# mako443/Text2Pos-CVPR2022

Measured on AMD Instinct MI355X. Metric: cells+queries encoded/sec and top-k retrieval QPS, 256-pt cells, 12k-cell DB, higher is better.
Workload: dtype f16x3 (fp32 operands split hi+lo into fp16, 3 f16 MFMAs, fp32 accumulate; fp32-class error) for the encoders / f64 MFMA for the ranking

## Files before the change

include/t2p.h:

```cpp
#ifndef T2P_H
#define T2P_H
#include <stddef.h>
#include <stdint.h>

#ifdef __cplusplus
extern "C" {
#endif

#define T2P_ABI_VERSION 29
#define T2P_DEFAULT_CHUNK_OBJECTS 65000
#define T2P_MAX_CHUNK_OBJECTS 65535
#define T2P_TUNING_MASK 0x1
#define T2P_E_ARG (-1)
#define T2P_E_WORKSPACE (-2)
#define T2P_E_UNSUPPORTED (-3)

typedef void* t2p_stream_t;

int t2p_abi_version(void);
const char* t2p_last_error(void);

typedef struct t2p_cell_weights {
    const float* sa_w1[3];
    const float* sa_b1[3];
    const float* sa_w2[3];
    const float* sa_b2[3];
    const float* ga_w1;
    const float* ga_b1;
    const float* ga_w2;
    const float* ga_b2;
    const float* lin1_w;
    const float* lin1_b;
    const float* lin2_w;
    const float* lin2_b;
    const float* pn_w;
    const float* pn_b;
    const float* col_w1;
    const float* col_b1;
    const float* col_w2;
    const float* col_b2;
    const float* pos_w1;
    const float* pos_b1;
    const float* pos_w2;
    const float* pos_b2;
    const float* merge_w;
    const float* merge_b;
    const float* g_wp;
    const float* g_bp;
    const float* g_wq;
    const float* g_w2;
    const float* g_b2;
    const float* lin_w1;
    const float* lin_b1;
    const float* lin_w2;
    const float* lin_b2;
    const void* sa_w2_x3[3];
    const void* ga_w2_x3;
    const float* sa_b2_x3[3];
    float sa_w2_scale[3];
    const void* lin1_x3;
    const void* lin2_x3;
    const void* merge_x3;
    const void* pn_x3;
    const void* g_wp_x3;
    const void* g_wq_x3;
    float lin1_scale, lin2_scale, merge_scale, pn_scale, g_wp_scale, g_wq_scale;
    const void* sa_w1_x3[3];
    const void* ga_w1_x3;
    const float* class_embedding;
    const float* color_embedding;
    float ga_w1_l1;
    float ga_b1_absmax;
    float sa_wp_l1[3];
    float sa_a1_l1;
    float sa_b1_absmax;
    const void* g_w2_x3;
} t2p_cell_weights;

typedef struct t2p_cell_config {
    int32_t n_pts;
    int32_t embed_dim;
    int32_t pointnet_features;
    int32_t use_class;
    int32_t use_color;
    int32_t use_position;
    int32_t self_loops;
    int32_t knn_k;
    int32_t variation;
    float radius[3];
    int32_t chunk_objects;
    int32_t precision;
    int32_t class_embed;
    int32_t color_embed;
    const int32_t* class_idx;
    const int32_t* color_idx;
// ... 159 lines not shown
```

text2pos-cvpr2022_amd/build.py:

```python
import os
import subprocess
import sys
from concurrent.futures import ThreadPoolExecutor

HERE = os.path.dirname(os.path.abspath(__file__))
CSRC = os.path.join(HERE, "csrc")
OBJ = os.path.join(CSRC, "_obj")
LIB = os.path.join(HERE, "libt2p_hip.so")
SOURCES = ["api.hip", "sample_group.hip", "small_kernels.hip", "tg_gemm.hip", "tg_gemm_tn.hip", "tg_gemm_x3.hip", "train_gemm.hip", "ws_gemm.hip", "ga2.hip", "ws_sa.hip", "sa_rows.hip", "sa3.hip", "sa_points.hip", "sa_x3.hip", "lstm.hip", "train_ops.hip", "sim_topk.hip", "match.hip", "classify.hip"]
HEADERS = [os.path.join(CSRC, "t2p_common.h"), os.path.join(HERE, "..", "include", "t2p.h")]
FLAGS = ["--offload-arch=gfx950", "-O3", "-std=c++17", "-fPIC", "-ffp-contract=off", "-Wall", "-Wno-unused-function"]


def _hipcc():
    for c in (os.environ.get("HIPCC"), "/opt/rocm/bin/hipcc", "hipcc"):
        if c and (os.path.sep not in c or os.path.exists(c)):
            return c
    raise RuntimeError("hipcc not found")


def _stale(target, deps):
    if not os.path.exists(target):
        return True
    t = os.path.getmtime(target)
    return any(os.path.getmtime(d) > t for d in deps)


def build_variant(name: str, defines, verbose: bool = False) -> str:
    global OBJ, LIB
    saved = (OBJ, LIB)
    OBJ, LIB = os.path.join(CSRC, "_obj_" + name), os.path.join(HERE, f"libt2p_hip_{name}.so")
    try:
        return build_hip(force=False, verbose=verbose, extra_flags=tuple("-D" + d for d in defines))
    finally:
        OBJ, LIB = saved


def build_hip(force: bool = False, verbose: bool = False, extra_flags=()) -> str:
    os.makedirs(OBJ, exist_ok=True)
    hipcc = _hipcc()
    jobs = []
    for s in SOURCES:
        src = os.path.join(CSRC, s)
        obj = os.path.join(OBJ, s.replace(".hip", ".o"))
        if force or _stale(obj, [src] + HEADERS):
            jobs.append([hipcc, *FLAGS, *extra_flags, "-c", src, "-o", obj])

    def run(cmd):
        if verbose:
            print(" ".join(cmd), flush=True)
        r = subprocess.run(cmd, capture_output=True, text=True)
        if r.returncode != 0:
            raise RuntimeError("hipcc failed: %s\n%s\n%s" % (" ".join(cmd), r.stdout, r.stderr))
        if verbose and r.stderr.strip():
            print(r.stderr)

    with ThreadPoolExecutor(max_workers=min(4, max(1, len(jobs)))) as ex:
        list(ex.map(run, jobs))
    objs = [os.path.join(OBJ, s.replace(".hip", ".o")) for s in SOURCES]
    if force or jobs or _stale(LIB, objs):
        run([hipcc, "--offload-arch=gfx950", "-shared", "-fPIC", "-Wl,--no-undefined", "-o", LIB, *objs])
    return LIB


def build_peaks() -> str:
    src = os.path.join(HERE, "..", "profiles", "microbench", "peaks.hip")
    lib = os.path.join(HERE, "..", "profiles", "microbench", "libt2p_peaks.so")
    if _stale(lib, [src]):
        r = subprocess.run([_hipcc(), "--offload-arch=gfx950", "-O3", "-std=c++17", "-fPIC", "-shared", "-o", lib, src],
                           capture_output=True, text=True)
        if r.returncode != 0:
            raise RuntimeError("hipcc failed on peaks.hip:\n" + r.stderr)
    return os.path.abspath(lib)


def build_host_ext() -> str:
    import sysconfig
    src = os.path.join(CSRC, "host_ext.c")
    lib = os.path.join(HERE, "_t2p_host" + (sysconfig.get_config_var("EXT_SUFFIX") or ".so"))
    if _stale(lib, [src]):
        cc = os.environ.get("CC") or "gcc"
        r = subprocess.run([cc, "-O3", "-std=gnu11", "-fPIC", "-shared", "-Wall", "-I" + sysconfig.get_paths()["include"], "-o", lib, src,
                            "-lpthread", "-lm"], capture_output=True, text=True)
        if r.returncode != 0:
            raise RuntimeError("building _t2p_host failed:\n" + r.stderr)
    return lib


if __name__ == "__main__":
    if "--variant" in sys.argv:
        i = sys.argv.index("--variant")
        print(build_variant(sys.argv[i + 1], sys.argv[i + 2:]))
# ... 5 lines not shown
```

text2pos-cvpr2022_amd/csrc/api.hip:

```cpp
#include <stdarg.h>
#include <stdlib.h>
#include <string.h>

#include <mutex>
#include <set>
#include <utility>

#include "../../include/t2p.h"
#include "t2p_common.h"

namespace t2p {

static thread_local char g_err[512] = "";

void set_error(const char* fmt, ...) {
    va_list ap;
    va_start(ap, fmt);
    vsnprintf(g_err, sizeof(g_err), fmt, ap);
    va_end(ap);
}

int num_cus() {
    static int cached = 0;
    if (cached == 0) {
// ... 157 lines not shown
        w.prefix[l] = b.take<int32_t>(n + 1);
        w.bounds[l] = b.take<int32_t>(1024 + 1);
    }
    w.seg_ptr = b.take<int32_t>(nb + 1);
    w.guard = b.take<uint32_t>(G_SLOTS);
    w.pool = b.take<float>(nb * D);
    w.l1 = b.take<float>(nb * D);
    w.l2 = b.take<float>(nb * D);
    if (ws) *ws = w;
    return align_up(b.off, 256);
}

int default_chunk(const t2p_cell_config& cfg) { return cfg.chunk_objects > 0 ? cfg.chunk_objects : T2P_DEFAULT_CHUNK_OBJECTS; }

int check_cfg(const t2p_cell_config* cfg) {
    T2P_CHECK_ARG(cfg != nullptr, "encode_cells: cfg is NULL");
    if (cfg->n_pts < 8 || cfg->n_pts > 256) {
        set_error("encode_cells: n_pts=%d not built (8 <= n_pts <= 256 points per object)", cfg->n_pts);
        return T2P_E_UNSUPPORTED;
    }
    if (cfg->objects_only) {
        if (cfg->embed_dim < 64 || cfg->embed_dim > 512 || cfg->embed_dim % 64 != 0) {
            set_error("encode_cells: objects_only supports embed_dim in {64, 128, ..., 512}, got %d", cfg->embed_dim);
            return T2P_E_UNSUPPORTED;
        }
    } else if (cfg->embed_dim != 256 && cfg->embed_dim != 128 && cfg->embed_dim != 384) {
        set_error("encode_cells: embed_dim=%d not built for the cell head (128, 256, 384; the host pads e.g. 300 to 384)", cfg->embed_dim);
        return T2P_E_UNSUPPORTED;
    }
    T2P_CHECK_ARG(cfg->variation == 0 || cfg->variation == 1, "encode_cells: variation=%d (0 = max, 1 = mean)",
                  cfg->variation);
    if (cfg->variation == 1 && cfg->knn_k != 8) {
        set_error("encode_cells: variation=1 (mean aggregation) is built for knn_k = 8 only, got %d", cfg->knn_k);
        return T2P_E_UNSUPPORTED;
    }
    T2P_CHECK_ARG(cfg->pointnet_features >= 0 && cfg->pointnet_features <= 2, "encode_cells: pointnet_features=%d",
                  cfg->pointnet_features);
    T2P_CHECK_ARG(cfg->use_class || cfg->use_color || cfg->use_position, "encode_cells: use_features is empty");
    T2P_CHECK_ARG(cfg->knn_k >= 1 && cfg->knn_k <= 32, "encode_cells: knn_k=%d outside [1,32]", cfg->knn_k);
    T2P_CHECK_ARG(cfg->precision == 0 || cfg->precision == 1, "encode_cells: precision=%d (0 = fp32, 1 = f16x3)",
                  cfg->precision);
    T2P_CHECK_ARG((cfg->tuning & ~T2P_TUNING_MASK) == 0, "encode_cells: tuning=%#x has bits outside %#x", cfg->tuning, T2P_TUNING_MASK);
    T2P_CHECK_ARG(cfg->chunk_objects >= 0 && cfg->chunk_objects <= T2P_MAX_CHUNK_OBJECTS,
                  "encode_cells: chunk_objects=%d outside [0, %d] (0 = default %d); the workspace takes ~0.6 MB per object of a chunk",
                  cfg->chunk_objects, T2P_MAX_CHUNK_OBJECTS, T2P_DEFAULT_CHUNK_OBJECTS);
    T2P_CHECK_ARG(!cfg->class_embed || cfg->class_idx != nullptr, "encode_cells: class_embed needs class_idx");
    T2P_CHECK_ARG(!cfg->color_embed || cfg->color_idx != nullptr, "encode_cells: color_embed needs color_idx");
    return 0;
}

template <typename T>
int copy_trace(T* dst, const T* src, size_t n, hipStream_t st) {
    if (dst == nullptr || n == 0) return 0;
    hipError_t e = hipMemcpyAsync(dst, src, n * sizeof(T), hipMemcpyDeviceToDevice, st);
    if (e != hipSuccess) {
        set_error("encode_cells: trace copy failed: %s", hipGetErrorString(e));
        return (int)e;
    }
    return 0;
}

int encode_chunk(const float* xyz, const float* rgb, const float* center, const float* mean_rgb,
                 const int32_t* cell_ptr_dev , int32_t o_lo, int64_t n, int64_t nb,
                 int max_cell, const t2p_cell_weights& W, const t2p_cell_config& cfg, float* out,
                 const t2p_cell_trace* tr, int64_t trace_obj0, CellWs& ws, hipStream_t st, bool trunk_only = false) {
    Geo g(cfg.n_pts);
    const int D = cfg.embed_dim;
    uint32_t* guard = (cfg.precision == 1 && cfg.overflow_flag != nullptr) ? ws.guard : nullptr;
    auto gslot = [&](int i) -> uint32_t* { return guard ? guard + i : nullptr; };
    GuardBounds gbounds{};
    for (int l = 0; l < 3; l++) gbounds.wp_l1[l] = W.sa_wp_l1[l];
    gbounds.a1_l1 = W.sa_a1_l1;
    gbounds.a1_bmax = W.sa_b1_absmax;
    gbounds.ga1_l1 = W.ga_w1_l1;
    gbounds.ga1_bmax = W.ga_b1_absmax;
    bool lds_btab[3];
    for (int l = 0; l < 3; l++) lds_btab[l] = cfg.precision == 1 && g.specialised(l);
    const bool sa1_points = lds_btab[0];
    if (trunk_only)
        T2P_TRY(launch_one_cell_index(n, ws.seg_ptr, ws.first, st, guard));
    else
        T2P_TRY(launch_cell_index(cell_ptr_dev, (int)nb, o_lo, ws.seg_ptr, ws.first, st, guard));
    const bool run_pointnet = cfg.use_class && !cfg.class_embed;
    if (run_pointnet) {
    ws.gt.self_loops = cfg.self_loops;
    {
        GroupTables gt = ws.gt;
        const bool want_nbr = tr != nullptr && (tr->nbr[0] || tr->nbr[1] || tr->nbr[2] || tr->cnt[0] || tr->cnt[1] || tr->cnt[2]);
        if (!want_nbr)
            for (int l = 0; l < 3; l++) gt.nbr[l] = gt.cnt[l] = nullptr;
        for (int l = 0; l < 3; l++) {
            const int cf = l == 0 ? 3 : Geo::C[l - 1];
            gt.B[l] = lds_btab[l] ? nullptr : ws.B[l];
            gt.wp[l] = W.sa_w1[l] + (size_t)cf * Geo::H[l];
            gt.H[l] = Geo::H[l];
            gt.tail[l] = ws.F[l];
            gt.ld_tail[l] = Geo::LD[l];
            gt.tail_col0[l] = Geo::C[l];
        }
        gt.tail_rows[2] = g.gp;
        gt.A1 = sa1_points ? nullptr : ws.A[0];
        gt.w1 = W.sa_w1[0];
        gt.b1 = W.sa_b1[0];
        gt.rgb = rgb;
        gt.H1 = Geo::H[0];
        gt.guard = guard;

        T2P_TRY(launch_sample_group(xyz, n, cfg.n_pts, cfg.radius, gt, st));
        if (!(cfg.tuning & 1) && cfg.n_pts == 256)
            T2P_TRY(launch_dedup_rows(xyz, rgb, n, cfg.n_pts, gt.rows[0], gt.n_rows[0], g.nc[0], st));
        SaParams bp[3] = {};
        for (int l = 0; l < 3; l++) {
            bp[l].n_rows = gt.n_rows[l];
            bp[l].n_obj = n;
            bp[l].prefix_ws = ws.prefix[l];
            bp[l].bounds_ws = ws.bounds[l];
            bp[l].W_x3 = cfg.precision == 1 ? W.sa_w2_x3[l] : nullptr;
            bp[l].wp = lds_btab[l] ? W.sa_w1[l] : nullptr;
            bp[l].n_dense = g.nd[l];
            bp[l].n_cent = g.nc[l];
        }
        bp[0].w1 = sa1_points ? W.sa_w1[0] : nullptr;
        T2P_TRY(launch_sa_balance_levels(bp, Geo::H, Geo::C, st));
    }

    for (int l = 0; l < 3; l++) {
        const int H = Geo::H[l], C = Geo::C[l];
        const int cf = l == 0 ? 3 : Geo::C[l - 1];
        const float* pos_src = l == 0 ? xyz : ws.F[l - 1];
        const int ld_pos = l == 0 ? 3 : Geo::LD[l - 1];
        const int pos_col0 = l == 0 ? 0 : Geo::C[l - 1];
        if (l != 0) {
            WsParams p{};
            p.A = ws.F[l - 1];
            p.lda = Geo::LD[l - 1];
            p.k_live = Geo::C[l - 1] + 4;
            p.W = W.sa_w1[l];
            p.W_x3 = cfg.precision == 1 ? W.sa_w1_x3[l] : nullptr;
            p.ldw = H;
            p.bias = W.sa_b1[l];
            p.out = ws.A[l];
            p.ldo = H;
            p.relu = 0;
            p.M = n * g.nd[l];
            p.amax_out = gslot(l == 1 ? G_A2 : G_A3);
            T2P_TRY(launch_ws(WS_DENSE_STORE, Geo::LD[l - 1] - (cfg.precision == 1 ? 16 : 0), H, p, st));
        }
        SaParams p{};
        p.A = ws.A[l];
        p.Bc = ws.B[l];
        p.wp = lds_btab[l] ? W.sa_w1[l] + (size_t)cf * Geo::H[l] : nullptr;
        p.W = W.sa_w2[l];
        p.W_x3 = cfg.precision == 1 ? W.sa_w2_x3[l] : nullptr;
        p.bias = cfg.precision == 1 ? W.sa_b2_x3[l] : W.sa_b2[l];
        p.out_scale = cfg.precision == 1 ? 1.0f / W.sa_w2_scale[l] : 1.0f;
        p.out = ws.F[l];
        p.ldo = Geo::LD[l];
        p.rows = ws.gt.rows[l];
        p.n_rows = ws.gt.n_rows[l];
        p.first = ws.first;
        p.fps_idx = ws.gt.fps_idx[l];
        p.pos_src = pos_src;
        p.ld_pos = ld_pos;
        p.pos_col0 = pos_col0;
        if (l == 0 && sa1_points) {
            p.feat_src = rgb;
            p.w1 = W.sa_w1[0];
            p.b1 = W.sa_b1[0];
        }
        p.n_dense = g.nd[l];
        p.n_cent = g.nc[l];
        p.n_obj = n;
        p.prefix_ws = ws.prefix[l];
        p.bounds_ws = ws.bounds[l];
        p.balanced = 1;
        p.amax_out = gslot(G_F1 + l);
        if (l == 2) p.out_rows = g.gp;
        T2P_TRY(launch_ws_sa(H, C, p, st));
    }
    {
        WsParams p{};
        p.A = ws.F[2];
        p.lda = Geo::LD[2];
        p.W = W.ga_w1;
        p.W_x3 = cfg.precision == 1 ? W.ga_w1_x3 : nullptr;
        p.ldw = 512;
        p.bias = W.ga_b1;
        p.out = ws.gh;
        _Float16* gh_hi = (_Float16*)ws.gh;
        _Float16* gh_lo = gh_hi + (size_t)gh_rows(n, g) * 512;
        if (cfg.precision == 1) {
            p.out_hi = gh_hi;
            p.out_lo = gh_lo;
            p.amax_out = gslot(G_GA_H);
        }
        p.ldo = 512;
        p.relu = 1;
        p.M = n * g.gp;
        T2P_TRY(launch_ws(WS_DENSE_STORE, Geo::LD[2] - (cfg.precision == 1 ? 16 : 0), 512, p, st));
        WsParams q{};
        q.A = ws.gh;
        if (cfg.precision == 1) {
            q.A_hi = gh_hi;
            q.A_lo = gh_lo;
        }
        q.lda = 512;
        q.W = W.ga_w2;
        q.W_x3 = cfg.precision == 1 ? W.ga_w2_x3 : nullptr;
        q.ldw = 1024;
        q.bias = W.ga_b2;
        q.out = ws.f0;
        q.ldo = 1024;
        q.relu = 1;
        q.M = n * g.gp;
        q.group_rows = g.gp;
        T2P_TRY(launch_ws(WS_DENSE_GROUPMAX, 512, 1024, q, st));
    }
    if (cfg.precision == 1 && W.lin1_x3 && W.lin2_x3) {
        T2P_TRY(launch_gemm_x3(ws.f0, 1024, W.lin1_x3, W.lin1_scale, W.lin1_b, ws.f1, 512, 0, n, 1024, 512, 1, st, nullptr, 0, gslot(G_PN_F0)));
        T2P_TRY(launch_gemm_x3(ws.f1, 512, W.lin2_x3, W.lin2_scale, W.lin2_b, ws.f2, 256, 0, n, 512, 256, 1, st, nullptr, 0, gslot(G_PN_F1)));
    } else {
        T2P_TRY(launch_gemm(ws.f0, 1024, W.lin1_w, W.lin1_b, ws.f1, 512, 0, n, 1024, 512, 1, st));
        T2P_TRY(launch_gemm(ws.f1, 512, W.lin2_w, W.lin2_b, ws.f2, 256, 0, n, 512, 256, 1, st));
    }
    }
    if (trunk_only) {
        T2P_TRY(copy_trace(tr->features0, ws.f0, (size_t)n * 1024, st));
        T2P_TRY(copy_trace(tr->features1, ws.f1, (size_t)n * 512, st));
        T2P_TRY(copy_trace(tr->features2, ws.f2, (size_t)n * 256, st));
        T2P_TRY(launch_guard_check(guard, cfg.overflow_flag, gbounds, st));
        return 0;
    }
    const int nfeat = (cfg.use_class ? 1 : 0) + (cfg.use_color ? 1 : 0) + (cfg.use_position ? 1 : 0);
    const int ldcat = nfeat * D;
    int slot = 0;
    if (cfg.use_class && cfg.class_embed) {
        T2P_TRY(launch_gather_rownorm(W.class_embedding, cfg.class_idx + o_lo, n, D, ws.cat, ldcat, slot * D, st));
        slot++;
    } else if (cfg.use_class) {
        const float* fin = cfg.pointnet_features == 0 ? ws.f0 : (cfg.pointnet_features == 1 ? ws.f1 : ws.f2);
        const int kin = cfg.pointnet_features == 0 ? 1024 : (cfg.pointnet_features == 1 ? 512 : 256);
        if (cfg.precision == 1 && W.pn_x3)
            T2P_TRY(launch_gemm_x3(fin, kin, W.pn_x3, W.pn_scale, W.pn_b, ws.P, D, 0, n, kin, D, 1, st, nullptr, 0,
                                          gslot(G_PN_F0 + cfg.pointnet_features)));
        else
            T2P_TRY(launch_gemm(fin, kin, W.pn_w, W.pn_b, ws.P, D, 0, n, kin, D, 1, st));
        T2P_TRY(launch_rownorm(ws.P, D, n, D, ws.cat, ldcat, slot * D, st));
        slot++;
    }
    if (cfg.use_color && cfg.color_embed) {
        T2P_TRY(launch_gather_rownorm(W.color_embedding, cfg.color_idx + o_lo, n, D, ws.cat, ldcat, slot * D, st));
        slot++;
    } else if (cfg.use_color) {
        T2P_TRY(launch_mlp3_norm(mean_rgb, n, W.col_w1, W.col_b1, W.col_w2, W.col_b2, D, ws.cat, ldcat, slot * D, st));
        slot++;
    }
    if (cfg.use_position) {
        T2P_TRY(launch_mlp3_norm(center, n, W.pos_w1, W.pos_b1, W.pos_w2, W.pos_b2, D, ws.cat, ldcat, slot * D, st));
        slot++;
    }
    const float* emb = ws.cat;
    if (nfeat > 1) {
        if (cfg.precision == 1 && W.merge_x3)
            T2P_TRY(launch_gemm_x3(ws.cat, ldcat, W.merge_x3, W.merge_scale, W.merge_b, ws.emb, D, 0, n, ldcat, D, 1, st, nullptr, 0, gslot(G_GEMM_IN)));
        else
            T2P_TRY(launch_gemm(ws.cat, ldcat, W.merge_w, W.merge_b, ws.emb, D, 0, n, ldcat, D, 1, st));
        emb = ws.emb;
    }
    if (cfg.objects_only) {
        T2P_TRY(copy_trace(tr->obj_emb + trace_obj0 * D, emb, (size_t)n * D, st));
        T2P_TRY(launch_guard_check(guard, cfg.overflow_flag, gbounds, st));
        return 0;
    }
    T2P_TRY(launch_rownorm(emb, D, n, D, ws.embn, D, 0, st));
    if (cfg.precision == 1 && W.g_wp_x3 && W.g_wq_x3) {
        T2P_TRY(launch_gemm_x3(ws.embn, D, W.g_wp_x3, W.g_wp_scale, W.g_bp, ws.P, D, 0, n, D, D, 0, st, nullptr, 0, gslot(G_GEMM_IN)));
        T2P_TRY(launch_gemm_x3(ws.embn, D, W.g_wq_x3, W.g_wq_scale, nullptr, ws.Q, D, 0, n, D, D, 0, st, nullptr, 0, gslot(G_GEMM_IN)));
    } else {
        T2P_TRY(launch_gemm(ws.embn, D, W.g_wp, W.g_bp, ws.P, D, 0, n, D, D, 0, st));
        T2P_TRY(launch_gemm(ws.embn, D, W.g_wq, nullptr, ws.Q, D, 0, n, D, D, 0, st));
    }
    T2P_TRY(launch_knn(ws.embn, D, ws.seg_ptr, (int)nb, max_cell, cfg.knn_k, ws.knn, st));
    {
        WsParams p{};
        p.A = ws.Q;
        p.lda = D;
        p.Bc = ws.P;
        p.W = W.g_w2;
        p.W_x3 = cfg.precision == 1 ? W.g_w2_x3 : nullptr;
        p.amax_out = gslot(G_EDGE);
        p.ldw = D;
        p.bias = W.g_b2;
        p.out = ws.x1;
        p.ldo = D;
        p.relu = 1;
        p.knn_group = (n + 31) / 32 < num_cus() ? 8 : 32;
        p.n_groups = (n + p.knn_group - 1) / p.knn_group;
        p.knn_idx = ws.knn;
        p.knn_k = cfg.knn_k;
        p.n_dst = n;
        p.mean = cfg.variation == 1;
        T2P_TRY(launch_ws(WS_EDGE_KNN, D, D, p, st));
    }
    T2P_TRY(launch_segmax(ws.x1, D, ws.seg_ptr, (int)nb, ws.pool, cfg.variation == 1, st));
    T2P_TRY(launch_gemm(ws.pool, D, W.lin_w1, W.lin_b1, ws.l1, D, 0, nb, D, D, 1, st));
    T2P_TRY(launch_gemm(ws.l1, D, W.lin_w2, W.lin_b2, ws.l2, D, 0, nb, D, D, 1, st));
    T2P_TRY(launch_rownorm(ws.l2, D, nb, D, out, D, 0, st));
    T2P_TRY(launch_guard_check(guard, cfg.overflow_flag, gbounds, st));

    if (tr && run_pointnet) {
        for (int l = 0; l < 3; l++) {
            T2P_TRY(copy_trace(tr->fps_idx[l] ? tr->fps_idx[l] + trace_obj0 * g.nc[l] : nullptr, ws.gt.fps_idx[l],
                               (size_t)n * g.nc[l], st));
            T2P_TRY(copy_trace(tr->nbr[l] ? tr->nbr[l] + trace_obj0 * g.nc[l] * 32 : nullptr, ws.gt.nbr[l],
                               (size_t)n * g.nc[l] * 32, st));
            T2P_TRY(copy_trace(tr->cnt[l] ? tr->cnt[l] + trace_obj0 * g.nc[l] : nullptr, ws.gt.cnt[l],
                               (size_t)n * g.nc[l], st));
            if (tr->sa_out[l] && n > 0) {
                const int rows = l == 2 ? g.gp : g.nc[l];
                const size_t ld = Geo::LD[l] * sizeof(float);
                hipError_t e = hipSuccess;
                if (rows == g.nc[l])
                    e = hipMemcpy2DAsync(tr->sa_out[l] + trace_obj0 * g.nc[l] * Geo::LD[l], ld, ws.F[l], ld, (Geo::C[l] + 4) * sizeof(float),
                                         (size_t)n * g.nc[l], hipMemcpyDeviceToDevice, st);
                for (int c = 0; rows != g.nc[l] && c < g.nc[l] && e == hipSuccess; c++)
                    e = hipMemcpy2DAsync(tr->sa_out[l] + (trace_obj0 * g.nc[l] + c) * Geo::LD[l], g.nc[l] * ld, ws.F[l] + (size_t)c * Geo::LD[l],
                                         rows * ld, (Geo::C[l] + 4) * sizeof(float), (size_t)n, hipMemcpyDeviceToDevice, st);
                if (e != hipSuccess) {
                    set_error("encode_cells: trace copy failed: %s", hipGetErrorString(e));
                    return (int)e;
                }
            }
        }
        T2P_TRY(copy_trace(tr->features0 ? tr->features0 + trace_obj0 * 1024 : nullptr, ws.f0, (size_t)n * 1024, st));
        T2P_TRY(copy_trace(tr->features1 ? tr->features1 + trace_obj0 * 512 : nullptr, ws.f1, (size_t)n * 512, st));
        T2P_TRY(copy_trace(tr->features2 ? tr->features2 + trace_obj0 * 256 : nullptr, ws.f2, (size_t)n * 256, st));
    }
    if (tr) {
        T2P_TRY(copy_trace(tr->obj_emb ? tr->obj_emb + trace_obj0 * D : nullptr, emb, (size_t)n * D, st));
        T2P_TRY(copy_trace(tr->knn_idx ? tr->knn_idx + trace_obj0 * cfg.knn_k : nullptr, ws.knn,
                           (size_t)n * cfg.knn_k, st));
    }
    return 0;
}

int64_t next_chunk_end(const int32_t* cp, int64_t c0, int64_t n_cells, int chunk) {
    int64_t c1 = c0 + 1;
    while (c1 < n_cells && (cp[c1 + 1] - cp[c0]) <= chunk) c1++;
    return c1;
}

}
}

using namespace t2p;

extern "C" {

int t2p_abi_version(void) { return T2P_ABI_VERSION; }

void t2p_profile_enable(int on) {
    std::lock_guard<std::mutex> lock(g_prof_mu);
    g_prof_on = on != 0;
// ... 537 lines not shown
```

text2pos-cvpr2022_amd/csrc/t2p_common.h:

```cpp
#pragma once
#include <hip/hip_runtime.h>
#include <stdint.h>
#include <stdio.h>

namespace t2p {

void set_error(const char* fmt, ...);

#define T2P_E_ARG (-1)
#define T2P_E_WORKSPACE (-2)
#define T2P_E_UNSUPPORTED (-3)

#define T2P_CHECK_ARG(cond, ...)                  \
    do {                                          \
        if (!(cond)) {                            \
            ::t2p::set_error(__VA_ARGS__);        \
            return T2P_E_ARG;                     \
        }                                         \
    } while (0)

#define T2P_CHECK_LAUNCH(name)                                                   \
    do {                                                                         \
        hipError_t e__ = hipGetLastError();                                      \
        if (e__ != hipSuccess) {                                                 \
// ... 81 lines not shown
    if ((threadIdx.x & 63) == 0) {
        const uint32_t b = __float_as_uint(m);
        if (b > __atomic_load_n(slot, __ATOMIC_RELAXED)) atomicMax(slot, b);
    }
}
__device__ __forceinline__ void guard_track_bits(uint32_t& acc, int lane_bits ) {
#pragma unroll
    for (int o = 32; o > 0; o >>= 1) {
        const int other = __shfl_xor(lane_bits, o, 64);
        lane_bits = other > lane_bits ? other : lane_bits;
    }
    const uint32_t b = (uint32_t)__builtin_amdgcn_readfirstlane(lane_bits);
    acc = b > acc ? b : acc;
}
#endif
int launch_guard_check(const uint32_t* guard, int32_t* overflow_flag, const GuardBounds& b, hipStream_t st);

struct ProfScope {
    ProfScope(const char* name, hipStream_t st);
    ~ProfScope();
    int slot;
    hipStream_t st;
    void* ev_end;
    int reps;
};
#define T2P_REPEAT(ps) for (int rep_ = (ps).reps; rep_ > 0; --rep_)

struct GroupTables {
    uint8_t* fps_idx[3];
    uint8_t* nbr[3];
    uint8_t* cnt[3];
    uint16_t* rows[3];
    uint16_t* n_rows[3];
    int self_loops;
    int n_dense[3];
    int n_cent[3];
    float* B[3];
    const float* wp[3];
    int H[3];
    float* tail[3];
    int ld_tail[3], tail_col0[3];
    int tail_rows[3];
    float* A1;
    const float* w1;
    const float* b1;
    const float* rgb;
    int H1;
    uint32_t* guard;
};
int launch_sample_group(const float* xyz, int64_t n_obj, int n_pts, const float radius[3], GroupTables gt,
                        hipStream_t st);
int launch_dedup_rows(const float* xyz, const float* rgb, int64_t n_obj, int n_pts, uint16_t* rows, uint16_t* n_rows,
                      int n_cent, hipStream_t st);

int launch_rownorm(const float* in, int ld_in, int64_t n_rows, int dim, float* out, int ld_out, int col0,
                   hipStream_t st);
int launch_gather_rownorm(const float* table, const int32_t* idx, int64_t n_rows, int dim, float* out, int ld_out,
                          int col0, hipStream_t st);
int launch_segmax(const float* in, int dim, const int32_t* seg_ptr, int n_seg, float* out, int mean,
                  hipStream_t st);
int launch_knn(const float* x, int dim, const int32_t* seg_ptr, int n_seg, int max_seg_rows, int k,
               int32_t* out_idx, hipStream_t st);
int launch_mlp3_norm(const float* in3, int64_t n_rows, const float* w1, const float* b1, const float* w2,
                     const float* b2, int D, float* out, int ld_out, int col0, hipStream_t st);
int launch_pack_objects(const float* raw_xyz, const float* raw_rgb, const int32_t* obj_ptr, const int32_t* sample_idx,
                        const float* rot, int64_t n_obj, int n_pts, float* xyz, float* rgb, float* center, float* mean_rgb,
                        hipStream_t st);
int launch_pack_scene(const float* raw_xyz, const float* raw_rgb, const int32_t* obj_ptr, const int32_t* obj_id, const uint64_t* key,
                      const float* scene_center, const float* scene_color, int64_t n_out, int n_pts, float* xyz, float* rgb,
                      float* center, float* mean_rgb, int32_t* idx_out, hipStream_t st);
int launch_pairwise_ranking(const float* scores, int batch, float margin, float* row_loss, float* d_scores, float* row_cnt,
                            hipStream_t st);
int launch_hardest_ranking(const float* scores, int batch, float margin, float* best, int32_t* where, float* d_scores,
                           hipStream_t st);
int launch_cell_index(const int32_t* cell_ptr, int n_cells, int32_t o_lo, int32_t* seg_ptr_local, int32_t* first,
                      hipStream_t st, uint32_t* guard_to_clear = nullptr);

int launch_gemm(const float* A, int lda, const float* W, const float* bias, float* C, int ldc, int c0, int64_t M,
                int K, int N, int relu, hipStream_t st, const float* resid = nullptr, int ldr = 0);
int launch_gemm_skinny(const float* A, int lda, const float* W, float* C, int ldc, int64_t M, int K, int N, hipStream_t st);
int launch_gemm_x3(const float* A, int lda, const void* Wx, float scale, const float* bias, float* C, int ldc, int c0,
                   int64_t M, int K, int N, int relu, hipStream_t st, const float* resid = nullptr, int ldr = 0,
                   uint32_t* amax_in = nullptr );

size_t gemm_tn_workspace_bytes(int64_t M, int K1, int N);
int launch_edge_counts(const uint16_t* rows, const uint16_t* n_rows, const int32_t* first_obj, int64_t n_obj, int n_dense, int n_cent,
                       int self_loops, int32_t* counts, hipStream_t st);
int launch_edge_expand(const uint16_t* rows, const uint16_t* n_rows, const int32_t* first_obj, const int32_t* cent_ptr, int64_t n_obj,
                       int n_dense, int n_cent, int self_loops, int32_t* src, int32_t* dst, hipStream_t st);
size_t linear_wgrad_workspace_bytes(int64_t M, int K1, int N);
int launch_linear_wgrad_f32(const float* dY, int lda, const float* X, int ldb, float* dW, int ldc, float* colsum, int64_t M, int K1, int N,
                            void* ws, size_t ws_bytes, hipStream_t st);
int launch_gemm_tn(const float* A, int lda, const float* B, int ldb, float* C, int ldc, int64_t M, int K1, int N, void* ws,
                   size_t ws_bytes, hipStream_t st);

enum WsMode { WS_DENSE_STORE = 0, WS_DENSE_GROUPMAX = 1, WS_EDGE_KNN = 3 };
struct WsParams {
    const float* A;
    int lda;
    int k_live;
    const float* Bc;
    const float* W;
    int ldw;
    const void* W_x3;
    const void* A_hi;
    const void* A_lo;
    void* out_hi;
    void* out_lo;
    const float* bias;
    float* out;
    int ldo;
    int relu;
    int64_t n_groups;
    int64_t M;
    uint32_t* amax_out;
    const int32_t* knn_idx;
    int knn_k;
    int64_t n_dst;
    int mean;
    int knn_group;
    int group_rows;
};
int launch_ws(int mode, int K, int N, const WsParams& p, hipStream_t st);

struct SaParams {
    const float* A;
    const float* Bc;
    const float* wp;
    const float* W;
    const void* W_x3;
    const float* bias;
    float out_scale;
    float* out;
    int ldo;
    const uint16_t* rows;
    const uint16_t* n_rows;
    const int32_t* first;
    const uint8_t* fps_idx;
    const float* pos_src;
    int ld_pos, pos_col0;
    const float* feat_src;
    const float* w1;
    const float* b1;
    int n_dense, n_cent;
    int64_t n_obj;
    int32_t* prefix_ws;
    int32_t* bounds_ws;
    int balanced;
    uint32_t* amax_out;
    int out_rows;
};
int launch_ws_sa(int H, int C, const SaParams& p, hipStream_t st);
int launch_sa_x3(int H, int C, const SaParams& p, hipStream_t st);
int sa_x3_launch_shape(int H, int C, int64_t n_obj, int* tile_rows, int* n_wg);
bool sa_rows_selected(int H, int C, const SaParams& p);
int launch_sa_rows(int H, int C, const SaParams& p, hipStream_t st);
int sa_rows_launch_shape(int64_t n_obj, int* tile_rows, int* n_wg);
bool sa_points_selected(int H, int C, const SaParams& p);
int launch_sa_points(int H, int C, const SaParams& p, hipStream_t st);
int sa_points_launch_shape(int64_t n_obj, int* tile_rows, int* n_wg);
bool sa3_selected(int H, int C, const SaParams& p);
int launch_sa3(const SaParams& p, hipStream_t st);
int sa3_launch_shape(int64_t n_obj, int* tile_rows, int* n_wg);
int launch_sa_balance_levels(const SaParams p[3], const int H[3], const int C[3], hipStream_t st);

int launch_bilstm_impl(const float* gate_table , const float* whh ,
// ... 43 lines not shown
```

Measured before the change: 151,300.

## Fuse per-object head MLPs, feature merge, norms and P/Q projections into one kernel

Adds a single persistent kernel that runs the whole per-object head in one pass over a row tile kept in LDS as split fp16 hi/lo planes. The fused stages are lin1, lin2, the pointnet projection and row norm, the color and position MLPs with norm, the merge GEMM and norm, and the P/Q projections. It replaces roughly ten separate launches and their global-memory intermediates (f1, f2, cat). It is enabled by default for the fp16x3, D=256 configuration, and tuning bit 4 turns it off. In exchange it needs a large LDS footprint per block, uses one block per CU with many barriers, and has a complex hand-written pipeline that could run slower than the tuned separate GEMMs.

```diff
diff --git a/include/t2p.h b/include/t2p.h
--- a/include/t2p.h
+++ b/include/t2p.h
@@ -10,7 +10,7 @@
 #define T2P_ABI_VERSION 29
 #define T2P_DEFAULT_CHUNK_OBJECTS 65000
 #define T2P_MAX_CHUNK_OBJECTS 65535
-#define T2P_TUNING_MASK 0x1
+#define T2P_TUNING_MASK 0x5
 #define T2P_E_ARG (-1)
 #define T2P_E_WORKSPACE (-2)
 #define T2P_E_UNSUPPORTED (-3)
diff --git a/text2pos-cvpr2022_amd/build.py b/text2pos-cvpr2022_amd/build.py
--- a/text2pos-cvpr2022_amd/build.py
+++ b/text2pos-cvpr2022_amd/build.py
@@ -7,7 +7,7 @@
 CSRC = os.path.join(HERE, "csrc")
 OBJ = os.path.join(CSRC, "_obj")
 LIB = os.path.join(HERE, "libt2p_hip.so")
-SOURCES = ["api.hip", "sample_group.hip", "small_kernels.hip", "tg_gemm.hip", "tg_gemm_tn.hip", "tg_gemm_x3.hip", "train_gemm.hip", "ws_gemm.hip", "ga2.hip", "ws_sa.hip", "sa_rows.hip", "sa3.hip", "sa_points.hip", "sa_x3.hip", "lstm.hip", "train_ops.hip", "sim_topk.hip", "match.hip", "classify.hip"]
+SOURCES = ["api.hip", "sample_group.hip", "small_kernels.hip", "tg_gemm.hip", "tg_gemm_tn.hip", "tg_gemm_x3.hip", "object_head.hip", "train_gemm.hip", "ws_gemm.hip", "ga2.hip", "ws_sa.hip", "sa_rows.hip", "sa3.hip", "sa_points.hip", "sa_x3.hip", "lstm.hip", "train_ops.hip", "sim_topk.hip", "match.hip", "classify.hip"]
 HEADERS = [os.path.join(CSRC, "t2p_common.h"), os.path.join(HERE, "..", "include", "t2p.h")]
 FLAGS = ["--offload-arch=gfx950", "-O3", "-std=c++17", "-fPIC", "-ffp-contract=off", "-Wall", "-Wno-unused-function"]
 
diff --git a/text2pos-cvpr2022_amd/csrc/api.hip b/text2pos-cvpr2022_amd/csrc/api.hip
--- a/text2pos-cvpr2022_amd/csrc/api.hip
+++ b/text2pos-cvpr2022_amd/csrc/api.hip
@@ -263,6 +263,10 @@
     else
         T2P_TRY(launch_cell_index(cell_ptr_dev, (int)nb, o_lo, ws.seg_ptr, ws.first, st, guard));
     const bool run_pointnet = cfg.use_class && !cfg.class_embed;
+    const bool fused_head = !(cfg.tuning & 4) && !trunk_only && !cfg.objects_only && cfg.precision == 1 && D == 256 && run_pointnet &&
+                            cfg.pointnet_features == 2 && cfg.use_color && !cfg.color_embed && cfg.use_position &&
+                            !(tr && (tr->features1 || tr->features2)) && W.lin1_x3 && W.lin2_x3 && W.pn_x3 && W.merge_x3 &&
+                            W.g_wp_x3 && W.g_wq_x3;
     if (run_pointnet) {
     ws.gt.self_loops = cfg.self_loops;
     {
@@ -397,7 +401,8 @@
         q.group_rows = g.gp;
         T2P_TRY(launch_ws(WS_DENSE_GROUPMAX, 512, 1024, q, st));
     }
-    if (cfg.precision == 1 && W.lin1_x3 && W.lin2_x3) {
+    if (fused_head) {
+    } else if (cfg.precision == 1 && W.lin1_x3 && W.lin2_x3) {
         T2P_TRY(launch_gemm_x3(ws.f0, 1024, W.lin1_x3, W.lin1_scale, W.lin1_b, ws.f1, 512, 0, n, 1024, 512, 1, st, nullptr, 0, gslot(G_PN_F0)));
         T2P_TRY(launch_gemm_x3(ws.f1, 512, W.lin2_x3, W.lin2_scale, W.lin2_b, ws.f2, 256, 0, n, 512, 256, 1, st, nullptr, 0, gslot(G_PN_F1)));
     } else {
@@ -414,6 +419,22 @@
     }
     const int nfeat = (cfg.use_class ? 1 : 0) + (cfg.use_color ? 1 : 0) + (cfg.use_position ? 1 : 0);
     const int ldcat = nfeat * D;
+    const float* emb = ws.cat;
+    if (fused_head) {
+        ObjectHeadArgs a{};
+        a.f0 = ws.f0; a.center = center; a.mean_rgb = mean_rgb; a.M = n;
+        a.lin1_x3 = W.lin1_x3; a.lin2_x3 = W.lin2_x3; a.pn_x3 = W.pn_x3; a.merge_x3 = W.merge_x3; a.wp_x3 = W.g_wp_x3; a.wq_x3 = W.g_wq_x3;
+        a.lin1_scale = W.lin1_scale; a.lin2_scale = W.lin2_scale; a.pn_scale = W.pn_scale; a.merge_scale = W.merge_scale;
+        a.wp_scale = W.g_wp_scale; a.wq_scale = W.g_wq_scale;
+        a.lin1_b = W.lin1_b; a.lin2_b = W.lin2_b; a.pn_b = W.pn_b; a.merge_b = W.merge_b; a.bp = W.g_bp;
+        a.col_w1 = W.col_w1; a.col_b1 = W.col_b1; a.col_w2 = W.col_w2; a.col_b2 = W.col_b2;
+        a.pos_w1 = W.pos_w1; a.pos_b1 = W.pos_b1; a.pos_w2 = W.pos_w2; a.pos_b2 = W.pos_b2;
+        a.emb = (tr && tr->obj_emb) ? ws.emb : nullptr;
+        a.embn = ws.embn; a.P = ws.P; a.Q = ws.Q;
+        a.g_f0 = gslot(G_PN_F0); a.g_f1 = gslot(G_PN_F1); a.g_f2 = gslot(G_PN_F2); a.g_in = gslot(G_GEMM_IN);
+        T2P_TRY(launch_object_head(a, st));
+        emb = ws.emb;
+    } else {
     int slot = 0;
     if (cfg.use_class && cfg.class_embed) {
         T2P_TRY(launch_gather_rownorm(W.class_embedding, cfg.class_idx + o_lo, n, D, ws.cat, ldcat, slot * D, st));
@@ -440,7 +461,6 @@
         T2P_TRY(launch_mlp3_norm(center, n, W.pos_w1, W.pos_b1, W.pos_w2, W.pos_b2, D, ws.cat, ldcat, slot * D, st));
         slot++;
     }
-    const float* emb = ws.cat;
     if (nfeat > 1) {
         if (cfg.precision == 1 && W.merge_x3)
             T2P_TRY(launch_gemm_x3(ws.cat, ldcat, W.merge_x3, W.merge_scale, W.merge_b, ws.emb, D, 0, n, ldcat, D, 1, st, nullptr, 0, gslot(G_GEMM_IN)));
@@ -460,6 +480,7 @@
     } else {
         T2P_TRY(launch_gemm(ws.embn, D, W.g_wp, W.g_bp, ws.P, D, 0, n, D, D, 0, st));
         T2P_TRY(launch_gemm(ws.embn, D, W.g_wq, nullptr, ws.Q, D, 0, n, D, D, 0, st));
+    }
     }
     T2P_TRY(launch_knn(ws.embn, D, ws.seg_ptr, (int)nb, max_cell, cfg.knn_k, ws.knn, st));
     {
diff --git a/text2pos-cvpr2022_amd/csrc/object_head.hip b/text2pos-cvpr2022_amd/csrc/object_head.hip
--- /dev/null
+++ b/text2pos-cvpr2022_amd/csrc/object_head.hip
@@ -0,0 +1,420 @@
+#include "t2p_common.h"
+
+namespace t2p {
+namespace {
+
+typedef _Float16 half8 __attribute__((ext_vector_type(8)));
+
+constexpr int NT = 512;
+constexpr int D = 256;
+constexpr int KC = 64;
+constexpr int LDS_ST = KC + 8;
+constexpr int LD1 = 512 + 8;
+constexpr int LD2 = D + 8;
+constexpr int LDY = D + 4;
+
+template <int RT>
+struct OhCfg {
+    static constexpr int MI = RT / 32;
+    static constexpr int FPT = RT * KC / NT;
+    static constexpr size_t kStage = (size_t)2 * 2 * RT * LDS_ST * sizeof(_Float16);
+    static constexpr size_t kPlanes512 = (size_t)2 * RT * LD1 * sizeof(_Float16);
+    static constexpr size_t kPlanes256 = (size_t)2 * RT * LD2 * sizeof(_Float16);
+    static constexpr size_t kOffY = kPlanes256;
+    static constexpr size_t kOffHid = kOffY + (size_t)RT * LDY * sizeof(float);
+    static constexpr size_t kOffSs = kOffHid + (size_t)RT * 64 * sizeof(float);
+    static constexpr size_t kEnd = kOffSs + (size_t)4 * RT * sizeof(float);
+    static constexpr size_t kLds = kEnd > kPlanes512 ? kEnd : kPlanes512;
+    static_assert(kStage <= kPlanes512 && kLds <= 160 * 1024, "object head: LDS plan");
+};
+
+struct OhParams {
+    const float* f0;
+    const float* center;
+    const float* mean_rgb;
+    int64_t M;
+    const _Float16 *lin1, *lin2, *pn, *merge, *wp, *wq;
+    float lin1_is, lin2_is, pn_is, merge_is, wp_is, wq_is;
+    const float *lin1_b, *lin2_b, *pn_b, *merge_b, *bp;
+    const float *col_w1, *col_b1, *col_w2, *col_b2, *pos_w1, *pos_b1, *pos_w2, *pos_b2;
+    float* emb;
+    float *embn, *P, *Q;
+    uint32_t *g_f0, *g_f1, *g_f2, *g_in;
+};
+
+typedef uint32_t u32x4 __attribute__((ext_vector_type(4)));
+__device__ __forceinline__ __amdgpu_buffer_rsrc_t weight_rsrc(const void* base, uint32_t bytes) {
+    return __builtin_amdgcn_make_buffer_rsrc((void*)base, 0, (int)bytes, 0x00020000);
+}
+template <int NJ>
+__device__ __forceinline__ void load_b(half8 (&b)[4][NJ][2], __amdgpu_buffer_rsrc_t w, uint32_t voff, uint32_t soff, uint32_t lo_bytes, int kp) {
+#pragma unroll
+    for (int s = 0; s < 4; s++)
+#pragma unroll
+        for (int j = 0; j < NJ; j++) {
+            const uint32_t so = soff + (uint32_t)j * 64 * kp;
+            b[s][j][0] = __builtin_bit_cast(half8, __builtin_amdgcn_raw_buffer_load_b128(w, voff + s * 32, so, 0));
+            b[s][j][1] = __builtin_bit_cast(half8, __builtin_amdgcn_raw_buffer_load_b128(w, voff + s * 32, so + lo_bytes, 0));
+        }
+}
+
+template <int MI, int NJ>
+__device__ __forceinline__ void mma_group(f32x16 (&acc)[MI][NJ], const _Float16* a, int a_lo, int lda, const half8 (&b)[4][NJ][2]) {
+#pragma unroll
+    for (int s = 0; s < 4; s++) {
+        half8 ah[MI], al[MI];
+#pragma unroll
+        for (int i = 0; i < MI; i++) {
+            const _Float16* p = a + i * 32 * lda + s * 16;
+            ah[i] = *(const half8*)p;
+            al[i] = *(const half8*)(p + a_lo);
+        }
+#pragma unroll
+        for (int i = 0; i < MI; i++)
+#pragma unroll
+            for (int j = 0; j < NJ; j++) {
+                acc[i][j] = __builtin_amdgcn_mfma_f32_32x32x16_f16(ah[i], b[s][j][0], acc[i][j], 0, 0, 0);
+                acc[i][j] = __builtin_amdgcn_mfma_f32_32x32x16_f16(ah[i], b[s][j][1], acc[i][j], 0, 0, 0);
+                acc[i][j] = __builtin_amdgcn_mfma_f32_32x32x16_f16(al[i], b[s][j][0], acc[i][j], 0, 0, 0);
+            }
+    }
+}
+
+template <int MI, int NJ>
+__device__ __forceinline__ void mma_seg(f32x16 (&acc)[MI][NJ], const _Float16* a, int a_lo, int lda, const _Float16* w, uint32_t soff,
+                                        uint32_t lo_bytes, int kp, int groups, int lane) {
+    const uint32_t voff = (uint32_t)((lane & 31) * kp + (lane >> 5) * 8) * 2u;
+    const __amdgpu_buffer_rsrc_t rs = weight_rsrc(w, 2 * lo_bytes);
+    half8 b0[4][NJ][2], b1[4][NJ][2];
+    load_b<NJ>(b0, rs, voff, soff, lo_bytes, kp);
+#pragma unroll 1
+    for (int g = 0; g < groups; g += 2) {
+        load_b<NJ>(b1, rs, voff, soff + (g + 1) * KC * 2, lo_bytes, kp);
+        mma_group<MI, NJ>(acc, a + g * KC, a_lo, lda, b0);
+        if (g + 2 < groups) load_b<NJ>(b0, rs, voff, soff + (g + 2) * KC * 2, lo_bytes, kp);
+        mma_group<MI, NJ>(acc, a + (g + 1) * KC, a_lo, lda, b1);
+    }
+}
+
+template <int MI, int NJ>
+__device__ __forceinline__ void zero_acc(f32x16 (&acc)[MI][NJ]) {
+#pragma unroll
+    for (int i = 0; i < MI; i++)
+#pragma unroll
+        for (int j = 0; j < NJ; j++)
+#pragma unroll
+            for (int e = 0; e < 16; e++) acc[i][j][e] = 0.f;
+}
+
+__device__ __forceinline__ void split_store(_Float16* hi_plane, int lo_off, int idx, float v) {
+    const _Float16 hi = (_Float16)v;
+    hi_plane[idx] = hi;
+    hi_plane[lo_off + idx] = (_Float16)(v - (float)hi);
+}
+
+template <int MI, int NJ>
+__device__ __forceinline__ void epi_planes(const f32x16 (&acc)[MI][NJ], float inv, const float* __restrict__ bias, int n0,
+                                           _Float16* hi_plane, int lo_off, int ld, int rows_live, float& gmax, int lane) {
+    const int h = lane >> 5, l31 = lane & 31;
+#pragma unroll
+    for (int j = 0; j < NJ; j++) {
+        const int col = n0 + j * 32 + l31;
+        const float bv = bias[col];
+#pragma unroll
+        for (int i = 0; i < MI; i++)
+#pragma unroll
+            for (int e = 0; e < 16; e++) {
+                const int r = i * 32 + (e & 3) + 8 * (e >> 2) + 4 * h;
+                const float v = fmaxf(fmaf(acc[i][j][e], inv, bv), 0.f);
+                if (r < rows_live) gmax = fmaxf(gmax, v);
+                split_store(hi_plane, lo_off, r * ld + col, v);
+            }
+    }
+}
+
+template <int MI>
+__device__ __forceinline__ void epi_f32(const f32x16 (&acc)[MI][1], float inv, const float* __restrict__ bias, int n0, float* Y, int lane) {
+    const int h = lane >> 5, l31 = lane & 31;
+    const int col = n0 + l31;
+    const float bv = bias[col];
+#pragma unroll
+    for (int i = 0; i < MI; i++)
+#pragma unroll
+        for (int e = 0; e < 16; e++) {
+            const int r = i * 32 + (e & 3) + 8 * (e >> 2) + 4 * h;
+            Y[r * LDY + col] = fmaxf(fmaf(acc[i][0][e], inv, bv), 0.f);
+        }
+}
+
+template <int RT>
+__device__ __forceinline__ void rownorm_rows(const float* Y, _Float16* hi_plane, int lo_off, int64_t row0, int rows_live, float* raw,
+                                             float* out, float& gmax, int lane, int wave) {
+#pragma unroll 1
+    for (int r = wave; r < RT; r += NT / 64) {
+        const float* x = Y + r * LDY;
+        float xv[D / 64];
+        float ss = 0.f;
+#pragma unroll
+        for (int j = 0; j < D / 64; j++) {
+            xv[j] = x[lane + 64 * j];
+            ss = fmaf(xv[j], xv[j], ss);
+        }
+#pragma unroll
+        for (int off = 32; off >= 1; off >>= 1) ss += __shfl_xor(ss, off, 64);
+        const float nrm = sqrtf(ss);
+        const float den = nrm > 1e-12f ? nrm : 1e-12f;
+        const bool live = r < rows_live;
+#pragma unroll
+        for (int j = 0; j < D / 64; j++) {
+            const float y = xv[j] / den;
+            split_store(hi_plane, lo_off, r * LD2 + lane + 64 * j, y);
+            if (live) {
+                gmax = fmaxf(gmax, fabsf(y));
+                if (raw) raw[(row0 + r) * D + lane + 64 * j] = xv[j];
+                if (out) out[(row0 + r) * D + lane + 64 * j] = y;
+            }
+        }
+    }
+}
+
+template <int RT>
+__device__ __forceinline__ void mlp_hidden(float* hid, const float* __restrict__ in3, const float* __restrict__ w1,
+                                           const float* __restrict__ b1, int64_t row0, int rows_live, int tid) {
+#pragma unroll 1
+    for (int i = tid; i < RT * 64; i += NT) {
+        const int r = i >> 6, u = i & 63;
+        float hv = 0.f;
+        if (r < rows_live) {
+            const float* x = in3 + (row0 + r) * 3;
+            float a = b1[u];
+            a = fmaf(x[0], w1[u], a);
+            a = fmaf(x[1], w1[64 + u], a);
+            a = fmaf(x[2], w1[128 + u], a);
+            hv = fmaxf(a, 0.f);
+        }
+        hid[i] = hv;
+    }
+}
+
+template <int RT>
+__device__ __forceinline__ void mlp_out_norm(const float* hid, float* ss, const float* __restrict__ w2, const float* __restrict__ b2,
+                                             _Float16* hi_plane, int lo_off, int rows_live, float& gmax, int tid) {
+    constexpr int R2 = RT / 2;
+    const int c = tid & (D - 1), r0 = (tid >> 8) * R2, cw = (tid >> 6) & 3;
+    float o[R2];
+    const float bv = b2[c];
+#pragma unroll
+    for (int r = 0; r < R2; r++) o[r] = bv;
+#pragma unroll 1
+    for (int k = 0; k < 64; k += 4) {
+        const float w0 = w2[k * D + c], w1 = w2[(k + 1) * D + c], w2_ = w2[(k + 2) * D + c], w3 = w2[(k + 3) * D + c];
+#pragma unroll
+        for (int r = 0; r < R2; r++) {
+            const f32x4 hv = *(const f32x4*)(hid + (r0 + r) * 64 + k);
+            o[r] = fmaf(hv[0], w0, o[r]);
+            o[r] = fmaf(hv[1], w1, o[r]);
+            o[r] = fmaf(hv[2], w2_, o[r]);
+            o[r] = fmaf(hv[3], w3, o[r]);
+        }
+    }
+#pragma unroll
+    for (int r = 0; r < R2; r++) {
+        o[r] = fmaxf(o[r], 0.f);
+        float v = fmaf(o[r], o[r], 0.f);
+#pragma unroll
+        for (int off = 32; off >= 1; off >>= 1) v += __shfl_xor(v, off, 64);
+        if ((tid & 63) == 0) ss[cw * RT + r0 + r] = v;
+    }
+    __syncthreads();
+#pragma unroll
+    for (int r = 0; r < R2; r++) {
+        const int rr = r0 + r;
+        const float nrm = sqrtf((ss[rr] + ss[RT + rr]) + (ss[2 * RT + rr] + ss[3 * RT + rr]));
+        const float y = o[r] / (nrm > 1e-12f ? nrm : 1e-12f);
+        if (rr < rows_live) gmax = fmaxf(gmax, y);
+        split_store(hi_plane, lo_off, rr * LD2 + c, y);
+    }
+}
+
+template <int RT>
+__global__ __launch_bounds__(NT) void k_object_head(const OhParams p, int64_t n_tiles) {
+    using Cf = OhCfg<RT>;
+    constexpr int MI = Cf::MI, FPT = Cf::FPT, TPR = KC / FPT;
+    extern __shared__ __attribute__((aligned(16))) unsigned char smem[];
+    _Float16* const X = (_Float16*)smem;
+    float* const Y = (float*)(smem + Cf::kOffY);
+    float* const hid = (float*)(smem + Cf::kOffHid);
+    float* const ss = (float*)(smem + Cf::kOffSs);
+    constexpr int ST_PLANE = RT * LDS_ST, P512 = RT * LD1, P256 = RT * LD2;
+
+    const int tid = threadIdx.x;
+    const int wave = __builtin_amdgcn_readfirstlane(tid >> 6);
+    float gmax_f0 = 0.f, gmax_f1 = 0.f, gmax_f2 = 0.f, gmax_in = 0.f;
+
+    for (int64_t tile = blockIdx.x; tile < n_tiles; tile += gridDim.x) {
+        const int64_t row0 = tile * RT;
+        int t = tid;
+        asm volatile("" : "+v"(t));
+        const int lane = t & 63;
+        const int h = lane >> 5, l31 = lane & 31;
+        const int rows_live = (int)((p.M - row0) < RT ? (p.M - row0) : RT);
+
+        f32x16 acc1[MI][2];
+        zero_acc<MI, 2>(acc1);
+        {
+            const int s_row = t / TPR, s_k = (t % TPR) * FPT;
+            const bool a_ok = s_row < rows_live;
+            const float* a_ptr = p.f0 + (row0 + s_row) * 1024 + s_k;
+            const uint32_t w_lo = 512u * 1024 * 2, w0 = (uint32_t)wave * 64 * 1024 * 2;
+            const __amdgpu_buffer_rsrc_t w = weight_rsrc(p.lin1, 2 * w_lo);
+            const uint32_t voff = (uint32_t)(l31 * 1024 + h * 8) * 2u;
+            const _Float16* a_frag = X + l31 * LDS_ST + h * 8;
+            f32x4 ra[FPT / 4];
+            auto stage_load = [&](int c) {
+#pragma unroll
+                for (int i = 0; i < FPT / 4; i++) ra[i] = a_ok ? *(const f32x4*)(a_ptr + c * KC + 4 * i) : f32x4{0.f, 0.f, 0.f, 0.f};
+            };
+            auto stage_store = [&](int buf) {
+                _Float16* base = X + buf * 2 * ST_PLANE + s_row * LDS_ST + s_k;
+#pragma unroll
+                for (int i = 0; i < FPT / 4; i++) {
+                    const f32x4 v = ra[i];
+                    gmax_f0 = fmaxf(fmaxf(gmax_f0, fmaxf(fabsf(v[0]), fabsf(v[1]))), fmaxf(fabsf(v[2]), fabsf(v[3])));
+                    const t2p_fp16x2 h01 = cvt_pk_f16(v[0], v[1]), h23 = cvt_pk_f16(v[2], v[3]);
+                    const t2p_fp16x2 l01 = cvt_pk_f16(v[0] - (float)h01[0], v[1] - (float)h01[1]);
+                    const t2p_fp16x2 l23 = cvt_pk_f16(v[2] - (float)h23[0], v[3] - (float)h23[1]);
+                    uint2 ph, pl;
+                    ph.x = __builtin_bit_cast(uint32_t, h01); ph.y = __builtin_bit_cast(uint32_t, h23);
+                    pl.x = __builtin_bit_cast(uint32_t, l01); pl.y = __builtin_bit_cast(uint32_t, l23);
+                    *(uint2*)(base + 4 * i) = ph;
+                    *(uint2*)(base + ST_PLANE + 4 * i) = pl;
+                }
+            };
+            half8 b0[4][2][2], b1[4][2][2];
+            stage_load(0);
+            load_b<2>(b0, w, voff, w0, w_lo, 1024);
+            stage_store(0);
+            __syncthreads();
+#pragma unroll 1
+            for (int c = 0; c < 1024 / KC; c += 2) {
+                stage_load(c + 1);
+                load_b<2>(b1, w, voff, w0 + (c + 1) * KC * 2, w_lo, 1024);
+                mma_group<MI, 2>(acc1, a_frag, ST_PLANE, LDS_ST, b0);
+                stage_store(1);
+                __syncthreads();
+                const bool more = c + 2 < 1024 / KC;
+                if (more) {
+                    stage_load(c + 2);
+                    load_b<2>(b0, w, voff, w0 + (c + 2) * KC * 2, w_lo, 1024);
+                }
+                mma_group<MI, 2>(acc1, a_frag + 2 * ST_PLANE, ST_PLANE, LDS_ST, b1);
+                if (more) stage_store(0);
+                __syncthreads();
+            }
+            epi_planes<MI, 2>(acc1, p.lin1_is, p.lin1_b, wave * 64, X, P512, LD1, rows_live, gmax_f1, lane);
+        }
+        __syncthreads();
+
+        f32x16 acc[MI][1];
+        zero_acc<MI, 1>(acc);
+        mma_seg<MI, 1>(acc, X + l31 * LD1 + h * 8, P512, LD1, p.lin2, (uint32_t)wave * 32 * 512 * 2, 256u * 512 * 2, 512, 8, lane);
+        __syncthreads();
+        epi_planes<MI, 1>(acc, p.lin2_is, p.lin2_b, wave * 32, X, P256, LD2, rows_live, gmax_f2, lane);
+        mlp_hidden<RT>(hid, p.mean_rgb, p.col_w1, p.col_b1, row0, rows_live, t);
+        __syncthreads();
+
+        const _Float16* a256 = X + l31 * LD2 + h * 8;
+        const uint32_t wn = (uint32_t)wave * 32;
+        zero_acc<MI, 1>(acc);
+        mma_seg<MI, 1>(acc, a256, P256, LD2, p.pn, wn * 256 * 2, 256u * 256 * 2, 256, 4, lane);
+        epi_f32<MI>(acc, p.pn_is, p.pn_b, wave * 32, Y, lane);
+        __syncthreads();
+        rownorm_rows<RT>(Y, X, P256, row0, rows_live, nullptr, nullptr, gmax_in, lane, wave);
+        __syncthreads();
+
+        f32x16 accm[MI][1];
+        zero_acc<MI, 1>(accm);
+        const uint32_t wm = wn * 768 * 2, wm_lo = 256u * 768 * 2;
+        mma_seg<MI, 1>(accm, a256, P256, LD2, p.merge, wm, wm_lo, 768, 4, lane);
+        __syncthreads();
+        mlp_out_norm<RT>(hid, ss, p.col_w2, p.col_b2, X, P256, rows_live, gmax_in, t);
+        mlp_hidden<RT>(hid, p.center, p.pos_w1, p.pos_b1, row0, rows_live, t);
+        __syncthreads();
+        mma_seg<MI, 1>(accm, a256, P256, LD2, p.merge, wm + 256 * 2, wm_lo, 768, 4, lane);
+        __syncthreads();
+        mlp_out_norm<RT>(hid, ss, p.pos_w2, p.pos_b2, X, P256, rows_live, gmax_in, t);
+        __syncthreads();
+        mma_seg<MI, 1>(accm, a256, P256, LD2, p.merge, wm + 512 * 2, wm_lo, 768, 4, lane);
+        epi_f32<MI>(accm, p.merge_is, p.merge_b, wave * 32, Y, lane);
+        __syncthreads();
+        rownorm_rows<RT>(Y, X, P256, row0, rows_live, p.emb, p.embn, gmax_in, lane, wave);
+        __syncthreads();
+
+        {
+            f32x16 accp[MI][2];
+            zero_acc<MI, 2>(accp);
+            const bool is_q = wave >= 4;
+            const int n0 = (wave & 3) * 64;
+            mma_seg<MI, 2>(accp, a256, P256, LD2, is_q ? p.wq : p.wp, (uint32_t)n0 * 256 * 2, 256u * 256 * 2, 256, 4, lane);
+            const float inv = is_q ? p.wq_is : p.wp_is;
+            float* outp = is_q ? p.Q : p.P;
+#pragma unroll
+            for (int j = 0; j < 2; j++) {
+                const int col = n0 + j * 32 + l31;
+                const float bv = is_q ? 0.f : p.bp[col];
+#pragma unroll
+                for (int i = 0; i < MI; i++)
+#pragma unroll
+                    for (int e = 0; e < 16; e++) {
+                        const int r = i * 32 + (e & 3) + 8 * (e >> 2) + 4 * h;
+                        if (r < rows_live) outp[(row0 + r) * D + col] = fmaf(accp[i][j][e], inv, bv);
+                    }
+            }
+        }
+        __syncthreads();
+    }
+    guard_publish_exact(p.g_f0, gmax_f0);
+    guard_publish_exact(p.g_f1, gmax_f1);
+    guard_publish_exact(p.g_f2, gmax_f2);
+    guard_publish_exact(p.g_in, gmax_in);
+}
+
+}
+
+int launch_object_head(const ObjectHeadArgs& a, hipStream_t st) {
+    T2P_CHECK_ARG(a.f0 && a.center && a.mean_rgb && a.embn && a.P && a.Q && a.lin1_x3 && a.lin2_x3 && a.pn_x3 && a.merge_x3 && a.wp_x3 &&
+                      a.wq_x3 && a.lin1_b && a.lin2_b && a.pn_b && a.merge_b && a.bp && a.col_w1 && a.col_b1 && a.col_w2 && a.col_b2 &&
+                      a.pos_w1 && a.pos_b1 && a.pos_w2 && a.pos_b2,
+                  "object_head: NULL argument");
+    T2P_CHECK_ARG(a.lin1_scale > 0.f && a.lin2_scale > 0.f && a.pn_scale > 0.f && a.merge_scale > 0.f && a.wp_scale > 0.f && a.wq_scale > 0.f,
+                  "object_head: weight image scales must be positive");
+    T2P_CHECK_ARG(((((uintptr_t)a.f0) | ((uintptr_t)a.lin1_x3) | ((uintptr_t)a.lin2_x3) | ((uintptr_t)a.pn_x3) | ((uintptr_t)a.merge_x3) |
+                    ((uintptr_t)a.wp_x3) | ((uintptr_t)a.wq_x3)) & 15) == 0,
+                  "object_head: f0 and the weight images must be 16-byte aligned");
+    if (a.M == 0) return 0;
+    OhParams p{};
+    p.f0 = a.f0; p.center = a.center; p.mean_rgb = a.mean_rgb; p.M = a.M;
+    p.lin1 = (const _Float16*)a.lin1_x3; p.lin2 = (const _Float16*)a.lin2_x3; p.pn = (const _Float16*)a.pn_x3;
+    p.merge = (const _Float16*)a.merge_x3; p.wp = (const _Float16*)a.wp_x3; p.wq = (const _Float16*)a.wq_x3;
+    p.lin1_is = 1.0f / a.lin1_scale; p.lin2_is = 1.0f / a.lin2_scale; p.pn_is = 1.0f / a.pn_scale;
+    p.merge_is = 1.0f / a.merge_scale; p.wp_is = 1.0f / a.wp_scale; p.wq_is = 1.0f / a.wq_scale;
+    p.lin1_b = a.lin1_b; p.lin2_b = a.lin2_b; p.pn_b = a.pn_b; p.merge_b = a.merge_b; p.bp = a.bp;
+    p.col_w1 = a.col_w1; p.col_b1 = a.col_b1; p.col_w2 = a.col_w2; p.col_b2 = a.col_b2;
+    p.pos_w1 = a.pos_w1; p.pos_b1 = a.pos_b1; p.pos_w2 = a.pos_w2; p.pos_b2 = a.pos_b2;
+    p.emb = a.emb; p.embn = a.embn; p.P = a.P; p.Q = a.Q;
+    p.g_f0 = a.g_f0; p.g_f1 = a.g_f1; p.g_f2 = a.g_f2; p.g_in = a.g_in;
+    ProfScope ps_("object_head", st);
+    const int64_t tiles32 = (a.M + 31) / 32, tiles64 = (a.M + 63) / 64;
+    if (tiles32 < num_cus()) {
+        T2P_TRY(reserve_lds((const void*)k_object_head<32>, OhCfg<32>::kLds, "object_head"));
+        hipLaunchKernelGGL(k_object_head<32>, dim3((unsigned)tiles32), dim3(NT), OhCfg<32>::kLds, st, p, tiles32);
+    } else {
+        T2P_TRY(reserve_lds((const void*)k_object_head<64>, OhCfg<64>::kLds, "object_head"));
+        const unsigned grid = (unsigned)(tiles64 < num_cus() ? tiles64 : num_cus());
+        hipLaunchKernelGGL(k_object_head<64>, dim3(grid), dim3(NT), OhCfg<64>::kLds, st, p, tiles64);
+    }
+    T2P_CHECK_LAUNCH("object_head");
+    return 0;
+}
+
+}
diff --git a/text2pos-cvpr2022_amd/csrc/t2p_common.h b/text2pos-cvpr2022_amd/csrc/t2p_common.h
--- a/text2pos-cvpr2022_amd/csrc/t2p_common.h
+++ b/text2pos-cvpr2022_amd/csrc/t2p_common.h
@@ -187,6 +187,21 @@
 int launch_gemm_x3(const float* A, int lda, const void* Wx, float scale, const float* bias, float* C, int ldc, int c0,
                    int64_t M, int K, int N, int relu, hipStream_t st, const float* resid = nullptr, int ldr = 0,
                    uint32_t* amax_in = nullptr );
+
+struct ObjectHeadArgs {
+    const float* f0;
+    const float* center;
+    const float* mean_rgb;
+    int64_t M;
+    const void *lin1_x3, *lin2_x3, *pn_x3, *merge_x3, *wp_x3, *wq_x3;
+    float lin1_scale, lin2_scale, pn_scale, merge_scale, wp_scale, wq_scale;
+    const float *lin1_b, *lin2_b, *pn_b, *merge_b, *bp;
+    const float *col_w1, *col_b1, *col_w2, *col_b2, *pos_w1, *pos_b1, *pos_w2, *pos_b2;
+    float* emb;
+    float *embn, *P, *Q;
+    uint32_t *g_f0, *g_f1, *g_f2, *g_in;
+};
+int launch_object_head(const ObjectHeadArgs& a, hipStream_t st);
 
 size_t gemm_tn_workspace_bytes(int64_t M, int K1, int N);
 int launch_edge_counts(const uint16_t* rows, const uint16_t* n_rows, const int32_t* first_obj, int64_t n_obj, int n_dense, int n_cent,
```

After: 151,500 (median of 3 runs). About the same (+0.1%).
